# qasimyu/simuscop

Hardware: AMD Instinct MI355X
Metric: simulated paired reads/sec (whole node) at 30x WGS PE150 (higher is better)
Workload: dtype u32

## Files before the change

simuscop_amd/csrc/sg_emit.h:

```cpp
#pragma once
#include "sg_device.h"
#include "sg_philox.h"

namespace sg {

#define EMIT_THREADS 1024
#define EMIT_WAVES (EMIT_THREADS / 64)
#define META_ROW 32

namespace row {
constexpr uint32_t kFlenMask = 0x3FFFFFFFu, kNpMax = 0xFFFFu, kNevMax = 63u, kHdrMax = 1023u;
constexpr uint32_t pack_x(uint32_t flen, uint32_t bad_block, uint32_t rev) { return flen | (bad_block << 30) | (rev << 31); }
constexpr uint32_t pack_y(uint32_t np, uint32_t nev, uint32_t hdr_len) { return np | (nev << 16) | (hdr_len << 22); }
constexpr uint32_t flen(uint32_t x) { return x & kFlenMask; }
constexpr uint32_t bad_block(uint32_t x) { return (x >> 30) & 1u; }
constexpr bool rev(uint32_t x) { return (x >> 31) != 0u; }
constexpr bool active(uint32_t x) { return (x & 0x7FFFFFFFu) != 0u; }
constexpr uint32_t np(uint32_t y) { return y & kNpMax; }
constexpr uint32_t nev(uint32_t y) { return (y >> 16) & kNevMax; }
constexpr uint32_t hdr_len(uint32_t y) { return y >> 22; }
constexpr uint32_t inv_of(uint32_t np) { return 0xFFFFFFFFu / np + 1u; }
constexpr uint32_t pack_src(uint32_t src_m5, bool rc) { return src_m5 | (rc ? 0x80000000u : 0u); }
constexpr uint32_t src_m5(uint32_t w) { return w & 0x7FFFFFFFu; }
constexpr bool copy_is_rc(uint32_t w) { return (w >> 31) != 0u; }

static_assert(np(pack_y(kNpMax, kNevMax, kHdrMax)) == kNpMax && nev(pack_y(kNpMax, kNevMax, kHdrMax)) == kNevMax &&
              hdr_len(pack_y(kNpMax, kNevMax, kHdrMax)) == kHdrMax, "m1.y: extreme values of all three fields");
static_assert(np(pack_y(kNpMax, 0, 0)) == kNpMax && nev(pack_y(kNpMax, 0, 0)) == 0 && hdr_len(pack_y(0, kNevMax, 0)) == 0 &&
              nev(pack_y(0, 0, kHdrMax)) == 0 && np(pack_y(0, kNevMax, kHdrMax)) == 0, "m1.y: no field leaks into a neighbour");
static_assert(flen(pack_x(kFlenMask, 1, 1)) == kFlenMask && bad_block(pack_x(kFlenMask, 1, 1)) == 1 && rev(pack_x(kFlenMask, 1, 1)),
              "m1.x: flen = 2^30 - 1 with both flag bits");
static_assert(bad_block(pack_x(kFlenMask, 0, 1)) == 0 && !rev(pack_x(kFlenMask, 1, 0)) && active(pack_x(1, 0, 0)) &&
              active(pack_x(0, 1, 0)) && !active(pack_x(0, 0, 1)), "m1.x: the flags are independent; rev alone is not active");
static_assert(src_m5(pack_src(0x7FFFFFFFu, true)) == 0x7FFFFFFFu && copy_is_rc(pack_src(0, true)) && !copy_is_rc(pack_src(0x7FFFFFFFu, false)),
              "m0.y of the straight-line kernel's row");
static_assert(inv_of(1) == 0u && inv_of(151) == 28443493u && inv_of(kNpMax) == 65538u, "ceil(2^32 / np) in 32 bits");
}

struct ReadRow {
  uint4 m0, m1;
  __device__ __forceinline__ static ReadRow load(const uint4* meta, size_t idx) { return ReadRow{meta[idx * 3], meta[idx * 3 + 1]}; }
  __device__ __forceinline__ static ReadRow none() { return ReadRow{make_uint4(0, 0, 0, 0), make_uint4(0, 0, 0, 0)}; }
  __device__ __forceinline__ static uint4 make_m0(uint64_t foff, uint32_t namepos, uint32_t fragcount) {
    return make_uint4((uint32_t)foff, (uint32_t)(foff >> 32), namepos, fragcount);
  }
  __device__ __forceinline__ static uint4 make_m1(uint32_t flen, uint32_t bad_block, uint32_t rev, uint32_t np, uint32_t nev,
                                                  uint32_t hdr_len, uint32_t event) {
    return make_uint4(row::pack_x(flen, bad_block, rev), row::pack_y(np, nev, hdr_len), row::inv_of(np), event);
  }
  __device__ __forceinline__ uint32_t flen() const { return row::flen(m1.x); }
  __device__ __forceinline__ bool rev() const { return row::rev(m1.x); }
  __device__ __forceinline__ uint32_t bad_block() const { return row::bad_block(m1.x); }
  __device__ __forceinline__ bool active() const { return row::active(m1.x); }
  __device__ __forceinline__ uint32_t np() const { return row::np(m1.y); }
// ... 197 lines not shown
```

simuscop_amd/csrc/sg_emit_fast.hip:

```cpp
#include "sg_emit.h"

namespace sg {

__device__ __forceinline__ uint32_t pack4(uint32_t w) {
  return (w | (w >> 6) | (w >> 12) | (w >> 18)) & 0xFFu;
}

typedef uint32_t u32x2 __attribute__((ext_vector_type(2)));
typedef uint32_t u32x4 __attribute__((ext_vector_type(4)));

#define FAST_CTX 192u

#define BITOP_OR_AND 0xF8
#define BITOP_XOR_AND 0x78
#define BITOP_ANDN_OR 0xBA

__device__ __noinline__ uint32_t tail_word(uint32_t slot, uint32_t c, uint32_t h, uint32_t c3b, uint32_t k0, uint32_t k1) {
  uint32_t y[4];
  philox_base(slot, 2u * c + (h >> 2), 1u, c3b, k0, k1, y);
  const uint32_t l = h & 3u;
  return l == 0u ? y[0] : l == 1u ? y[1] : l == 2u ? y[2] : y[3];
}

template <int H>
__device__ __forceinline__ void sample1(uint32_t col_sh, uint32_t col_mask, uint32_t cw, uint32_t wh, uint32_t so_h, uint32_t qo_h, uint32_t cd4_w,
                                        uint32_t& acc, uint32_t& sy) {
  typedef const __attribute__((address_space(3))) uint32_t* lds_word;
  const uint32_t kv4 = (cw >> (2 * H + 4)) & 0xFCu;
  const uint32_t keepm1 = *(lds_word)(uintptr_t)(so_h + kv4);
  const uint32_t d_s = keepm1 - (wh >> 16);
  const uint32_t col16 = (wh >> col_sh) & col_mask;
  const uint32_t qa = qo_h + ((cd4_w >> (8 * (H & 3))) & 0xFFu);
  const uint32_t e = *(lds_word)(uintptr_t)(qa + col16 + FAST_CTX * 4u);
  const uint32_t d_q = (wh & 0xFFFFu) - (e & 0xFFFFu);
  const uint32_t z = __builtin_amdgcn_bitop3_b32(d_q - 1u, d_q, d_s, BITOP_ANDN_OR);
  acc = __builtin_amdgcn_bitop3_b32(acc, z, 1u << (17 + H), BITOP_OR_AND);
  sy = __builtin_amdgcn_bitop3_b32(e >> 8, e, d_q, BITOP_XOR_AND);
}

__device__ __forceinline__ void sample8(const uint32_t* code4, uint32_t lgW, uint32_t cw, const uint32_t (&x)[8],
                                        const uint32_t (&so)[8], uint32_t qo0, uint32_t qo1, uint32_t (&sw)[2], uint32_t (&qw)[2],
                                        uint32_t& acc_out) {
  const uint32_t cd4[2] = {code4[(cw >> 10) & 0xFFu], code4[(cw >> 18) & 0xFFu]};
  const uint32_t col_sh = 12u - lgW, col_mask = ((1u << lgW) - 1u) << 4;
  uint32_t acc = 0, sy[8];
  sample1<0>(col_sh, col_mask, cw, x[0], so[0], qo0, cd4[0], acc, sy[0]);
  sample1<1>(col_sh, col_mask, cw, x[1], so[1], qo1, cd4[0], acc, sy[1]);
  sample1<2>(col_sh, col_mask, cw, x[2], so[2], so[2], cd4[0], acc, sy[2]);
  sample1<3>(col_sh, col_mask, cw, x[3], so[3], so[3], cd4[0], acc, sy[3]);
  sample1<4>(col_sh, col_mask, cw, x[4], so[4], so[4], cd4[1], acc, sy[4]);
  sample1<5>(col_sh, col_mask, cw, x[5], so[5], so[5], cd4[1], acc, sy[5]);
  sample1<6>(col_sh, col_mask, cw, x[6], so[6], so[6], cd4[1], acc, sy[6]);
  sample1<7>(col_sh, col_mask, cw, x[7], so[7], so[7], cd4[1], acc, sy[7]);
#pragma unroll
  for (int g = 0; g < 2; g++) {
    const uint32_t p01 = __builtin_amdgcn_perm(sy[4 * g + 1], sy[4 * g], 0x0C0C0602u);
    const uint32_t p23 = __builtin_amdgcn_perm(sy[4 * g + 3], sy[4 * g + 2], 0x06020C0Cu);
    qw[g] = p01 | p23;
    sw[g] = __builtin_amdgcn_perm(0u, 0x47544341u, cd4[g] >> 2);
  }
  acc_out = acc;
}

__device__ __forceinline__ void store_var(uint8_t* q, uint64_t lo, uint64_t hi, uint32_t n) {
  if (n >= 8u) {
    __builtin_memcpy(q, &lo, 8);
    if (n > 8u) {
      const uint32_t k = 8u * (n - 8u);
      const uint64_t v = (lo >> k) | (hi << (64u - k));
      __builtin_memcpy(q + n - 8u, &v, 8);
    }
  } else if (n >= 4u) {
    const uint32_t a = (uint32_t)lo, b = (uint32_t)(lo >> (8u * (n - 4u)));
    __builtin_memcpy(q, &a, 4);
    if (n > 4u) __builtin_memcpy(q + n - 4u, &b, 4);
  } else if (n >= 2u) {
    const uint16_t a = (uint16_t)lo, b = (uint16_t)(lo >> (8u * (n - 2u)));
    __builtin_memcpy(q, &a, 2);
    if (n > 2u) __builtin_memcpy(q + n - 2u, &b, 2);
  } else if (n == 1u) {
    *q = (uint8_t)lo;
  }
}

constexpr uint32_t FAST_G = 63u;

template <bool PAIRED, bool DIAG>
struct FastBlock {
  const DevProfile& P;
  const DevBatch& B;
  uint32_t m, tm;
  uint32_t dg;
  uint32_t bins, TI, inv_TI, clean_cap;
  uint32_t img_at;
  const uint32_t* lut;
  const uint32_t* code4;
  bool tail_whole;
  uint32_t TIp;
  uint32_t TI16, inv_TI16;

  __device__ __forceinline__ FastBlock(const DevProfile& P_, const DevBatch& B_, uint32_t m_, uint32_t TI_, uint32_t inv_TI_,
                                       uint32_t clean_cap_, uint32_t img_at_, const uint32_t* lut_, const uint32_t* code4_)
      : P(P_), B(B_), m(m_), tm(PAIRED ? m_ : 0u), dg(DIAG ? B_.diag : 0u), bins((uint32_t)P_.bins), TI(TI_), inv_TI(inv_TI_),
        clean_cap(clean_cap_), img_at(img_at_), lut(lut_), code4(code4_) {
    tail_whole = ((uint32_t)P.L & 7u) == 7u && ((uint32_t)P.L + 7u) / 8u == TI;
    TIp = tail_whole ? TI : TI - 1u;
    TI16 = (tail_whole ? TIp - 1u : TIp) >> 1;
    inv_TI16 = TI16 ? (1u << 20) / TI16 + 1u : 0u;
  }
  __device__ __forceinline__ bool rc(bool row_bit) const { return PAIRED ? m == 1u : row_bit; }
  __device__ __forceinline__ uint2 fetch_window(bool row_bit, uint32_t idx) const {
    uint2 v;
    fetch_window(row_bit, idx, v);
    return v;
// ... 22 lines not shown
  __device__ __forceinline__ unsigned long long lanes_below() const { return (1ull << lane) - 1ull; }
};

template <bool PAIRED, bool DIAG>
__device__ __forceinline__ void heads8(const FastBlock<PAIRED, DIAG>& k, uint32_t slot, uint32_t c, uint32_t (&x)[8]) {
  const uint32_t c3b = k.c3b();
  if (k.dg & 8u) {
#pragma unroll
    for (int z = 0; z < 8; z++) x[z] = (slot * 2654435761u) ^ (c * 40503u + z * 0x9E3779B9u);
  } else {
    philox_base(slot, 2u * c, 0, c3b, k.B.k0, k.B.k1, x);
    philox_base(slot, 2u * c + 1u, 0, c3b, k.B.k0, k.B.k1, x + 4);
  }
}

template <class S, class Fetch, class Run>
__device__ __forceinline__ void pipelined_steps(S cur, uint32_t first, uint32_t last, Fetch fetch, Run run) {
  for (uint32_t step = first; step < last; step++) {
    const S nxt = fetch(min(step + 1u, last - 1u));
    run(cur);
    cur = nxt;
  }
}

template <bool PAIRED, bool DIAG>
__device__ __forceinline__ void flush_slow(const FastBlock<PAIRED, DIAG>& k, FastWave& w) {
  const DevBatch& B = k.B;
  const uint32_t m = k.m, lane = w.lane;
  wave_lds_sync();
  uint32_t base = 0;
  if (lane == 0u) base = atomicAdd(B.slowq_count + m, w.nslow);
  base = (uint32_t)__builtin_amdgcn_readfirstlane((int)base);
  for (uint32_t b0 = 0; b0 < w.nslow; b0 += 64u) {
    const uint32_t i = b0 + lane;
    if (i < w.nslow && base + i < B.slowq_cap) {
      const uint32_t e = w.slow_list[i];
      B.slowq[(size_t)m * B.slowq_cap + base + i] = make_uint2(w.g * FAST_G + (e & 0xFFu), e >> 8);
    }
  }
  if (lane == 0u && base + w.nslow > B.slowq_cap) atomicOr((unsigned long long*)(B.totals + 3), 2ull);
  w.nslow = 0;
  wave_lds_sync();
}

template <bool PAIRED, bool DIAG>
__device__ __forceinline__ void flush_fix(const FastBlock<PAIRED, DIAG>& k, FastWave& w) {
  const DevProfile& P = k.P;
  const DevBatch& B = k.B;
  const uint32_t bins = k.bins, lane = w.lane;
  wave_lds_sync();
  __builtin_amdgcn_s_waitcnt(0x0F70);
  const uint32_t lgW = P.lgW, u_mask = (1u << (16u - lgW)) - 1u;
  const uint4* gsub = P.fast_sub + (size_t)k.tm * bins * FAST_CTX;
  const uint32_t c3b = k.c3b();
  for (uint32_t b0 = 0; b0 < w.nfix; b0 += 64u) {
    const uint2 fe = w.fix_list[b0 + lane < w.nfix ? b0 + lane : 0u];
    uint32_t todo = b0 + lane < w.nfix ? (fe.x >> 6) & 0xFFu : 0u;
    const uint32_t r = fe.x & 63u, c = fe.x >> 17, cw = fe.y;
    const uint32_t slot = w.g * FAST_G + r + B.slot_offset;
    const FastRow rr = w.rows.load(r);
    const uint32_t np = rr.np(), hl = rr.hdr_len();
    const bool whole = 8u * c + 8u <= np + (uint32_t)((np & 7u) == 7u);
    const uint32_t inv = row::inv_of(max(np, 1u));
    while (__ballot(todo != 0u) != 0ull) {
      const bool on = todo != 0u;
      const uint32_t h = on ? (uint32_t)__builtin_ctz(todo) : 0u;
      todo &= todo - 1u;
      const uint32_t i = 8u * c + h;
      const uint32_t bin = __umulhi(__umul24(i, bins), inv);
      uint32_t xw[4];
      philox_base(slot, 2u * c + (h >> 2), 0, c3b, B.k0, B.k1, xw);
      const uint32_t l = h & 3u;
      const uint32_t wh = l == 0u ? xw[0] : l == 1u ? xw[1] : l == 2u ? xw[2] : xw[3];
      const uint32_t region = c == 0u ? (h == 0u ? 128u : h == 1u ? 64u : 0u) : 0u;
      const uint32_t cdn = (cw >> (2u * h + 10u)) & 3u;
      const uint4 row = gsub[(size_t)bin * FAST_CTX + region + ((cw >> (2u * h + 6u)) & 63u)];
      const uint32_t sh = wh >> 16, h0 = row.x >> 16, h1 = row.y >> 16, h2 = row.z >> 16;
      const uint32_t jj = (uint32_t)(sh > h0) + (uint32_t)(sh > h1) + (uint32_t)(sh > h2);
      const bool amb_s = on && jj != (uint32_t)(sh >= h0) + (uint32_t)(sh >= h1) + (uint32_t)(sh >= h2);
      uint32_t kn = 0;
      uint2 e2 = make_uint2(0, 0);
      const uint32_t col = (wh & 0xFFFFu) >> (16u - lgW), uh = wh & u_mask;
      auto column = [&](uint32_t j_) {
        const uint32_t jm = max(j_, row.w & 3u);
        kn = (row.w >> (2u * jm + 2u)) & 3u;
        e2 = P.fast_alias[((((size_t)cdn * 4u + kn) * bins + bin) << lgW) + col];
      };
      if (!amb_s) column(jj);
      const bool need_tail = amb_s || (on && uh == (e2.x >> 16) && (e2.y & 0xFFu) != (e2.y >> 8));
      uint32_t wt = 0;
      if (__ballot(need_tail) != 0ull) {
        if (need_tail) wt = tail_word(slot, c, h, c3b, B.k0, B.k1);
      }
      if (__ballot(amb_s) != 0ull) {
        if (amb_s) {
          const uint32_t xs = (wh & 0xFFFF0000u) | (wt >> 16);
          column((uint32_t)(xs > row.x) + (uint32_t)(xs > row.y) + (uint32_t)(xs > row.z));
        }
      }
      const uint32_t th = e2.x >> 16;
      const bool lo_side = uh != th ? uh < th : ((uh << 16) | (wt & 0xFFFFu)) < e2.x;
      const uint32_t sym = (lo_side ? (e2.y & 0xFFu) : (e2.y >> 8)) + (uint32_t)P.min_qual;
      const uint32_t ch = (0x47544341u >> (8u * kn)) & 0xFFu;
      if (on) {
        if (whole) {
          uint8_t* rec = w.gout + rr.out_off() + hl + i;
          rec[0] = (uint8_t)ch;
          rec[np + 3u] = (uint8_t)sym;
        } else if (!rr.parked_slow()) {
          w.rows.patch_parked(r, h, ch, sym);
        }
      }
    }
  }
  w.nfix = 0;
  wave_lds_sync();
}

template <bool PAIRED, bool DIAG>
__device__ __forceinline__ void push_fix(const FastBlock<PAIRED, DIAG>& k, FastWave& w, uint32_t r, uint32_t c, uint32_t fix, uint32_t cw) {
  const unsigned long long fm = __ballot(fix != 0u);
  if (fm) {
    if (w.nfix + 64u > FIX_CAP) flush_fix(k, w);
    if (fix != 0u) w.fix_list[w.nfix + (uint32_t)__popcll(fm & w.lanes_below())] = make_uint2(r | (fix << 6) | (c << 17), cw);
    w.nfix += (uint32_t)__popcll(fm);
  }
}

__device__ __forceinline__ void stage_tables(const DevProfile& P, uint32_t tm, uint32_t TI, uint32_t* img, uint32_t img_at,
                                             uint32_t* lut, uint32_t* code4) {
  const uint32_t tid = threadIdx.x, bins = (uint32_t)P.bins, img_words = bins * P.fast_stride;
  const uint4* src = (const uint4*)(P.fast_lds + (size_t)tm * P.fast_mate_words);
  for (uint32_t i = tid; i < (img_words + 3u) / 4u; i += EMIT_THREADS) ((uint4*)img)[i] = src[i];
  const uint32_t blk_bytes = P.fast_stride * 4u;
  for (uint32_t i = tid; i < TI * LUT_ROW; i += EMIT_THREADS) {
    const uint32_t c = i / LUT_ROW, f = i - c * LUT_ROW;
    const uint32_t h = f < 8u ? f : f - 8u;
    const uint32_t pos = 8u * c + h;
    const uint32_t bin = min(pos * bins / (uint32_t)P.L, bins - 1u);
    uint32_t v = bin * blk_bytes;
    if (f < 8u && c == 0u) v += f == 0u ? 128u * 4u : f == 1u ? 64u * 4u : 0u;
    lut[i] = f < 10u ? v + img_at : 0u;
  }
  for (uint32_t i = tid; i < 256u; i += EMIT_THREADS) {
    uint32_t v = 0;
    for (uint32_t z = 0; z < 4u; z++) v |= (((i >> (2u * z)) & 3u) * 4u) << (8u * z);
    code4[i] = v;
  }
}

template <bool PAIRED>
__device__ __forceinline__ void store_name(const DevBatch& B, uint32_t m, const ReadRow& my, size_t idx, uint8_t* rec) {
  const uint32_t nv = my.hdr_len() - B.prefix_len;
  if (__builtin_expect(nv > 16u, 0)) {
    write_name(rec, B.prefix, B.prefix_len, my.namepos(), my.fragcount(), PAIRED ? 1u : 0u, m);
    return;
  }
  const uint64_t p_lo = ((uint64_t)B.prefix_w[1] << 32) | B.prefix_w[0], p_hi = ((uint64_t)B.prefix_w[3] << 32) | B.prefix_w[2];
  const uint4 tx = B.meta[idx * 3 + 2];
  const uint64_t b0 = ((uint64_t)tx.y << 32) | tx.x, b1 = ((uint64_t)tx.w << 32) | tx.z;
  const uint32_t plen = B.prefix_len, hb = plen + nv;
  if (plen < 16u && hb >= 16u && hb <= 24u) {
    const uint32_t sh = 8u * plen;
    uint64_t w0, w1, w2;
    if (sh < 64u) {
      w0 = p_lo | (b0 << sh);
      w1 = p_hi | (b1 << sh) | (sh ? b0 >> (64u - sh) : 0ull);
      w2 = sh ? b1 >> (64u - sh) : 0ull;
    } else {
      const uint32_t t2 = sh - 64u;
      w0 = p_lo;
      w1 = p_hi | (b0 << t2);
      w2 = (b1 << t2) | (t2 ? b0 >> (64u - t2) : 0ull);
    }
    struct { uint64_t a, b; } first = {w0, w1};
    __builtin_memcpy(rec, &first, 16);
    const uint32_t n2 = hb - 16u;
// ... 110 lines not shown
  {
    const uint32_t rem = gp.n_clean & 63u, idle = (0u - (gp.n_fast * TI + gp.n_single + gp.n_gen_all)) & 63u;
    if (rem != 0u && rem <= idle && gp.n_single + gp.n_gen_all + rem <= OVF_CAP) gp.n_moved = rem;
  }
  gp.n_ovf = gp.n_moved + gp.n_single + gp.n_gen_all;
  gp.more = (k.dg & 256u) ? 0ull : __ballot(gp.extra > 2u);
  return gp;
}

template <bool PAIRED, bool DIAG>
__device__ __forceinline__ void compose_lists(const FastBlock<PAIRED, DIAG>& k, const FastWave& w, GroupPlan& gp) {
  const uint32_t TI = k.TI, lane = w.lane, items = gp.items, n_moved = gp.n_moved;
  const unsigned long long lt = w.lanes_below();
  if (items > 0u && !gp.split_l) {
    if (gp.plain_l) {
      const uint32_t pos = (uint32_t)__popcll(gp.m_plain & lt);
      w.permp[pos] = (uint8_t)lane;
      if (!k.tail_whole) w.ovf[n_moved + pos] = (uint16_t)(lane | (k.TIp << 8));
    } else {
      uint32_t pos;
      if ((gp.m_rest >> lane) & 1ull) pos = (uint32_t)__popcll(gp.m_rest & lt);
      else if ((gp.m_one >> lane) & 1ull) pos = gp.n_rest + (uint32_t)__popcll(gp.m_one & lt);
      else pos = gp.n_rest + gp.n_one + (uint32_t)__popcll(gp.m_multi & lt);
      w.perm[pos] = (uint8_t)lane;
    }
  }
  if (gp.n_fast == 0u && lane == 0u) w.perm[0] = 0;
  if (gp.small) {
    const uint32_t o = n_moved + gp.n_psingle + (uint32_t)__popcll(gp.b1 & lt) + (uint32_t)__popcll(gp.b2 & lt);
    w.ovf[o] = (uint16_t)(lane | (TI << 8));
    if (gp.extra == 2u) w.ovf[o + 1u] = (uint16_t)(lane | ((TI + 1u) << 8));
  }
  if (gp.split_l) {
    const uint32_t kb = gp.kb, ka = gp.ka, ca0 = gp.ca0;
    const uint32_t oc = (gp.vscan >> 16) - (kb + ka);
    uint32_t og = n_moved + gp.n_single + (gp.vscan & 0xFFFFu) - gp.n_gen;
    const uint32_t kt = kb + ka, behind = ((ca0 - kb) << 7) | 64u;
    for (uint32_t q = 0; q < kt; q++) w.clean[oc + q] = (uint16_t)((lane | (q << 7)) + (q >= kb ? behind : 0u));
    const uint32_t mid_end = ka ? ca0 : items;
    for (uint32_t c = kb; c < mid_end; c++) w.ovf[og++] = (uint16_t)(lane | (c << 8));
    if (ka) for (uint32_t c = gp.n_whole; c < items; c++) w.ovf[og++] = (uint16_t)(lane | (c << 8));
  }
  wave_lds_sync();
  if (n_moved) {
    gp.n_clean -= n_moved;
    if (lane < n_moved) {
      const uint32_t e = w.clean[gp.n_clean + lane];
      w.ovf[lane] = (uint16_t)((e & 63u) | ((e >> 7) << 8));
    }
    wave_lds_sync();
  }
}

struct PlainSteps {
  bool use16;
  uint32_t n_plain, np16steps, cnt8, c8_base, n_pitems, npsteps;
};
template <bool PAIRED, bool DIAG>
__device__ __forceinline__ PlainSteps plan_plain_steps(const FastBlock<PAIRED, DIAG>& k, uint32_t n_plain) {
  PlainSteps ps;
  const uint32_t dg = k.dg, TIp = k.TIp, TI16 = k.TI16;
  ps.n_plain = n_plain;
  ps.use16 = !(dg & 512u) && TIp >= 18u;
  const uint32_t n_p16 = ps.use16 ? n_plain * TI16 : 0u;
  ps.np16steps = (dg & 128u) ? 0u : n_p16 >> 6;
  const uint32_t rem16 = n_p16 - (ps.np16steps << 6);
  ps.cnt8 = ps.use16 ? TIp - 2u * TI16 : TIp;
  ps.c8_base = ps.use16 ? 2u * TI16 : 0u;
  ps.n_pitems = 2u * rem16 + n_plain * ps.cnt8;
  ps.npsteps = (dg & 128u) ? 0u : (ps.n_pitems + 63u) / 64u;
  return ps;
}

__device__ __forceinline__ void lut_bins(const uint32_t* lut, uint32_t c, uint32_t (&so)[8], uint32_t& qo0, uint32_t& qo1) {
  const uint4* lrow = (const uint4*)(lut + c * LUT_ROW);
  const uint4 r0 = lrow[0], r1 = lrow[1], r2 = lrow[2];
  so[0] = r0.x; so[1] = r0.y; so[2] = r0.z; so[3] = r0.w; so[4] = r1.x; so[5] = r1.y; so[6] = r1.z; so[7] = r1.w;
  qo0 = r2.x; qo1 = r2.y;
}

struct P16 { uint32_t r, c, src, out; uint2 w; };

template <bool PAIRED, bool DIAG>
__device__ __forceinline__ void plain16_step(const FastBlock<PAIRED, DIAG>& k, FastWave& w, const P16& st, uint32_t qual_at) {
  const uint32_t dg = k.dg;
  const uint32_t c8 = 2u * st.c;
  const uint64_t w64 = window_codes(st.w, st.src);
  uint32_t cwa = (uint32_t)w64, cwb = (uint32_t)(w64 >> 16);
  const uint32_t slot = w.g * FAST_G + st.r + k.B.slot_offset;
  if (dg & 4u) { cwa = (w.g * FAST_G + st.r) * 2654435761u + c8; cwb = cwa * 40503u + 1u; }
  uint32_t sw[4], qw[4], fixv[2];
#pragma unroll
  for (int hf = 0; hf < 2; hf++) {
    uint32_t x[8];
    const uint32_t c = c8 + (uint32_t)hf, cw = hf ? cwb : cwa;
    heads8(k, slot, c, x);
    uint32_t so[8], qo0, qo1;
    lut_bins(k.lut, c, so, qo0, qo1);
    uint32_t s2[2], q2[2], acc;
    sample8(k.code4, k.P.lgW, cw, x, so, qo0, qo1, s2, q2, acc);
    sw[2 * hf] = s2[0]; sw[2 * hf + 1] = s2[1];
    qw[2 * hf] = q2[0]; qw[2 * hf + 1] = q2[1];
    fixv[hf] = (dg & 16u) ? 0u : (acc >> 17) & 0xFFu;
  }
  const uint32_t so_ = (dg & 1u) ? 0xFFFFFFFFu : st.out;
  const uint32_t qo_ = (dg & 1u) ? 0xFFFFFFFFu : st.out + qual_at;
  __builtin_amdgcn_raw_buffer_store_b128(u32x4{sw[0], sw[1], sw[2], sw[3]}, w.out_rsrc, so_, 0, 0);
  __builtin_amdgcn_raw_buffer_store_b128(u32x4{qw[0], qw[1], qw[2], qw[3]}, w.out_rsrc, qo_, 0, 0);
#pragma unroll
  for (int hf = 0; hf < 2; hf++) push_fix(k, w, st.r, c8 + (uint32_t)hf, fixv[hf], hf ? cwb : cwa);
}

template <bool PAIRED, bool DIAG>
__device__ __forceinline__ void plain16_steps(const FastBlock<PAIRED, DIAG>& k, FastWave& w, uint32_t a16, uint32_t b16) {
  uint32_t TI16_v = k.TI16, inv_TI16_v = k.inv_TI16, qual_at = (uint32_t)k.P.L + 3u;
  asm volatile("" : "+v"(TI16_v), "+v"(inv_TI16_v), "+v"(qual_at));
  auto fetch16 = [&](uint32_t step) -> P16 {
    P16 st;
    const uint32_t i = step * 64u + w.lane;
    const uint32_t ri = __umul24(i, inv_TI16_v) >> 20;
    st.c = i - __umul24(ri, TI16_v);
    st.r = w.permp[ri];
    const uint32_t A = w.rows.src_word(st.r);
    st.src = row::src_m5(A) + 16u * st.c;
    st.out = w.rows.base_off(st.r) + 16u * st.c;
    st.w = k.fetch_window(row::copy_is_rc(A), st.src);
    return st;
  };
  P16 cur = fetch16(a16);
  __builtin_amdgcn_raw_buffer_store_b128(u32x4{0u, 0u, 0u, 0u}, w.out_rsrc, 0xFFFFFFFFu, 0, 0);
  __builtin_amdgcn_raw_buffer_store_b128(u32x4{0u, 0u, 0u, 0u}, w.out_rsrc, 0xFFFFFFF0u, 0, 0);
  pipelined_steps(cur, a16, b16, fetch16, [&](const P16& st) { plain16_step(k, w, st, qual_at); });
}

template <bool PAIRED, bool DIAG>
__device__ __forceinline__ void sample_store8(const FastBlock<PAIRED, DIAG>& k, FastWave& w, uint32_t r, uint32_t c, bool ok, uint2 win,
                                              uint32_t src, const uint32_t (&so)[8], uint32_t qo0, uint32_t qo1, uint32_t out,
                                              uint32_t qual_at, bool tail_patch) {
  const uint32_t dg = k.dg;
  uint32_t cw;
  if (dg & 4u) cw = (w.g * FAST_G + r) * 2654435761u + c;
  else cw = (uint32_t)window_codes(win, src);
  uint32_t x[8];
  heads8(k, w.g * FAST_G + r + k.B.slot_offset, c, x);
  uint32_t sw[2], qw[2], acc;
  sample8(k.code4, k.P.lgW, cw, x, so, qo0, qo1, sw, qw, acc);
  const bool st_ok = ok && !(dg & 1u);
  const uint32_t so_ = st_ok ? out : 0xFFFFFFFFu;
  const uint32_t qo_ = st_ok ? out + qual_at : 0xFFFFFFFFu;
  uint32_t fix_mask = 0xFFu;
  if (tail_patch) {
    const bool last = c + 1u == k.TI;
    const uint32_t sel = last ? 0x04020100u : 0x03020100u;
    sw[1] = __builtin_amdgcn_perm(0x0Au, sw[1], sel);
    qw[1] = __builtin_amdgcn_perm(0x0Au, qw[1], sel);
    __builtin_amdgcn_raw_buffer_store_b16((unsigned short)0x0A2Bu, w.out_rsrc, st_ok && last ? so_ + 8u : 0xFFFFFFFFu, 0, 0);
    fix_mask = last ? 0x7Fu : 0xFFu;
  }
  __builtin_amdgcn_raw_buffer_store_b64(u32x2{sw[0], sw[1]}, w.out_rsrc, so_, 0, 0);
  __builtin_amdgcn_raw_buffer_store_b64(u32x2{qw[0], qw[1]}, w.out_rsrc, qo_, 0, 0);
  const uint32_t fix = (ok && !(dg & 16u)) ? (acc >> 17) & fix_mask : 0u;
  push_fix(k, w, r, c, fix, cw);
}

struct PStage { uint32_t r, c, src, out; bool ok; uint2 w; };

template <bool PAIRED, bool DIAG>
__device__ __forceinline__ void plain8_steps(const FastBlock<PAIRED, DIAG>& k, FastWave& w, const PlainSteps& ps, uint32_t a8, uint32_t b8) {
  const uint32_t cnt8 = ps.cnt8, c8_base = ps.c8_base, n_pitems = ps.n_pitems, TI16 = k.TI16, inv_TI16 = k.inv_TI16;
  uint32_t qual_at = (uint32_t)k.P.L + 3u, n_single = ps.n_plain * cnt8, i16_base = ps.np16steps << 6;
  asm volatile("" : "+v"(qual_at), "+v"(n_single), "+v"(i16_base));
  const uint32_t inv_cnt8 = cnt8 ? (1u << 20) / cnt8 + 1u : 0u;
  auto fetch_plain = [&](uint32_t step) -> PStage {
    PStage st;
    const uint32_t i_raw = step * 64u + w.lane;
    st.ok = i_raw < n_pitems;
    const uint32_t i = min(i_raw, n_pitems - 1u);
    const bool half = i >= n_single;
    const uint32_t j = i - n_single;
    const uint32_t q = half ? i16_base + (j >> 1) : i;
    const uint32_t d = half ? TI16 : cnt8;
    const uint32_t ri = __umul24(q, half ? inv_TI16 : inv_cnt8) >> 20;
    const uint32_t rem = q - __umul24(ri, d);
    st.c = half ? 2u * rem + (j & 1u) : c8_base + rem;
    st.r = w.permp[ri];
    const uint32_t A = w.rows.src_word(st.r);
    st.src = row::src_m5(A) + 8u * st.c;
    st.out = w.rows.base_off(st.r) + 8u * st.c;
    st.w = k.fetch_window(row::copy_is_rc(A), st.src);
    return st;
  };
  auto run_plain = [&](const PStage& st) {
    uint32_t so[8], qo0, qo1;
    lut_bins(k.lut, st.c, so, qo0, qo1);
    sample_store8(k, w, st.r, st.c, st.ok, st.w, st.src, so, qo0, qo1, st.out, qual_at, k.tail_whole);
  };
  PStage cur = fetch_plain(a8);
  __builtin_amdgcn_raw_buffer_store_b64(u32x2{0u, 0u}, w.out_rsrc, 0xFFFFFFFFu, 0, 0);
  __builtin_amdgcn_raw_buffer_store_b64(u32x2{0u, 0u}, w.out_rsrc, 0xFFFFFFF0u, 0, 0);
  if (k.tail_whole) __builtin_amdgcn_raw_buffer_store_b16((unsigned short)0u, w.out_rsrc, 0xFFFFFFE0u, 0, 0);
  pipelined_steps(cur, a8, b8, fetch_plain, run_plain);
}

template <bool PAIRED, bool DIAG>
__device__ __forceinline__ void plain_steps(const FastBlock<PAIRED, DIAG>& k, FastWave& w, uint32_t n_plain) {
  const PlainSteps ps = plan_plain_steps(k, n_plain);
  const uint32_t h16 = ps.np16steps >> 1, s8_first = (ps.use16 && ps.cnt8 && ps.npsteps) ? 1u : 0u;
#pragma unroll 1
  for (uint32_t ph = 0; ph < 2u; ph++) {
    const uint32_t a16 = ph ? h16 : 0u, b16 = ph ? ps.np16steps : h16;
    const uint32_t a8 = ph ? s8_first : 0u, b8 = ph ? ps.npsteps : s8_first;
    if (a16 < b16) plain16_steps(k, w, a16, b16);
    if (a8 < b8) plain8_steps(k, w, ps, a8, b8);
  }
}
// ... 136 lines not shown
    }
#pragma unroll 1
    for (; __ballot(q_ins <= q_end) != 0ull; q_ins++) {
      if (q_ins <= q_end) {
        const int p = (int)i0 - 5 + q_ins, ej = (int)(ie.ew_in & 0xFFFFu);
        const uint32_t prof = __umulhi(aux_draw(k.B, slot, ie.tj_in, (uint32_t)(p - ej), k.m), 3u);
        const uint32_t nat = (k.P.inv_remap_packed >> (2u * prof)) & 3u;
        cw = (cw & ~(3u << (2 * q_ins))) | (nat << (2 * q_ins));
      }
    }
  }
  return cw;
}

template <bool PAIRED, bool DIAG>
__device__ __forceinline__ void item_bins(const FastBlock<PAIRED, DIAG>& k, const Stage& st, uint32_t (&so)[8], uint32_t& qo0, uint32_t& qo1) {
  const uint32_t c = st.c, bins = k.bins, blk_bytes = k.P.fast_stride * 4u;
  const bool active = st.active;
  const bool lut_ok = st.row.np() == (uint32_t)k.P.L && c < k.TI;
  if (__ballot(active && !lut_ok) == 0ull) {
    lut_bins(k.lut, lut_ok ? c : 0u, so, qo0, qo1);
  } else {
    const uint32_t ib0 = __umul24(8u * c, bins), inv = st.row.inv();
#pragma unroll
    for (int h = 0; h < 8; h++) {
      const uint32_t bin = __umulhi(ib0 + (uint32_t)h * bins, inv);
      so[h] = __umul24(active ? bin : 0u, blk_bytes) + k.img_at;
    }
    qo0 = so[0]; qo1 = so[1];
    if (c == 0u) { so[0] += 128u * 4u; so[1] += 64u * 4u; }
  }
}

template <bool PAIRED, bool DIAG>
__device__ __forceinline__ void store_item(const FastBlock<PAIRED, DIAG>& k, const FastWave& w, const Stage& st, bool slow,
                                           const uint32_t (&sw)[2], const uint32_t (&qw)[2]) {
  const uint32_t np = st.row.np(), i0 = 8u * st.c;
  const bool active = st.active, go = active && !slow;
  const bool last7 = i0 + 7u == np;
  const bool whole = i0 + 8u <= np || last7;
  const bool sto = go && whole && !(k.dg & 1u);
  const uint32_t so_ = sto ? st.row.out_off() + st.row.hdr_len() + i0 : 0xFFFFFFFFu;
  const uint32_t qo_ = sto ? so_ + np + 3u : 0xFFFFFFFFu;
  const uint32_t s1 = last7 ? (sw[1] & 0x00FFFFFFu) | 0x0A000000u : sw[1];
  const uint32_t q1 = last7 ? (qw[1] & 0x00FFFFFFu) | 0x0A000000u : qw[1];
  __builtin_amdgcn_raw_buffer_store_b64(u32x2{sw[0], s1}, w.out_rsrc, so_, 0, 0);
  __builtin_amdgcn_raw_buffer_store_b64(u32x2{qw[0], q1}, w.out_rsrc, qo_, 0, 0);
  __builtin_amdgcn_raw_buffer_store_b16((unsigned short)0x0A2Bu, w.out_rsrc, sto && last7 ? so_ + 8u : 0xFFFFFFFFu, 0, 0);
  if (active && i0 + 8u > np && !(last7 && !slow)) w.rows.park(st.r, slow, sw, qw);
}

template <bool PAIRED, bool DIAG>
__device__ __forceinline__ bool fast_item(const FastBlock<PAIRED, DIAG>& k, const FastWave& w, const Stage& st, const ItemEvents& ie,
                                          uint32_t& fix, uint32_t& cw_out) {
  const bool active = st.active;
  const uint32_t c = st.c, slot = w.g * FAST_G + st.r;
  const uint32_t np = st.row.np(), nev = active ? ie.n_in : 0u;
  const uint32_t bad = st.row.bad_block();
  const uint32_t cw = item_codes(k, st, st.w, ie, nev, slot);
  uint32_t x[8];
  heads8(k, slot + k.B.slot_offset, c, x);
  uint32_t so[8], qo0, qo1;
  item_bins(k, st, so, qo0, qo1);
  uint32_t qw[2], sw[2], acc;
  sample8(k.code4, k.P.lgW, cw, x, so, qo0, qo1, sw, qw, acc);
  const bool slow = active && (bad != 0u || nev >= 2u);
  fix = (active && !slow && !(k.dg & 16u)) ? (acc >> 17) & 0xFFu & ((1u << min(8u, np - 8u * c)) - 1u) : 0u;
  cw_out = cw;
  store_item(k, w, st, slow, sw, qw);
  return slow;
}

template <bool PAIRED, bool DIAG>
__device__ __forceinline__ void general_step(const FastBlock<PAIRED, DIAG>& k, FastWave& w, const Stage& st) {
  const ItemEvents ie = item_events(k, w, st);
  uint32_t fix, cw;
  const bool slow = fast_item(k, w, st, ie, fix, cw);
  const unsigned long long sm = __ballot(slow);
  if (sm) {
    if (slow) w.slow_list[w.nslow + (uint32_t)__popcll(sm & w.lanes_below())] = st.r | (st.c << 8);
    w.nslow += (uint32_t)__popcll(sm);
  }
  push_fix(k, w, st.r, st.c, fix, cw);
}

template <bool PAIRED, bool DIAG>
__device__ __forceinline__ void general_steps(const FastBlock<PAIRED, DIAG>& k, FastWave& w, const GroupPlan& gp) {
  const uint32_t n_items = gp.n_fast * k.TI, n_stream = n_items + gp.n_ovf;
  const uint32_t nmain = (k.dg & 256u) ? 0u : (n_stream + 63u) / 64u;
  if (!nmain) return;
  Stage cur = fetch_step(k, w, n_items, n_stream, 0u);
  __builtin_amdgcn_raw_buffer_store_b64(u32x2{0u, 0u}, w.out_rsrc, 0xFFFFFFFFu, 0, 0);
  __builtin_amdgcn_raw_buffer_store_b64(u32x2{0u, 0u}, w.out_rsrc, 0xFFFFFFF0u, 0, 0);
  __builtin_amdgcn_raw_buffer_store_b16((unsigned short)0u, w.out_rsrc, 0xFFFFFFE0u, 0, 0);
  pipelined_steps(
      cur, 0u, nmain,
      [&](uint32_t step) {
        if (w.nslow > SLOW_CAP - 64u) flush_slow(k, w);
        return fetch_step(k, w, n_items, n_stream, step);
      },
      [&](const Stage& st) { general_step(k, w, st); });
}

template <bool PAIRED, bool DIAG>
__device__ __forceinline__ void past_map_steps(const FastBlock<PAIRED, DIAG>& k, FastWave& w, unsigned long long more) {
  uint32_t cb = k.TI;
  while (more) {
    if (w.nslow > SLOW_CAP - 64u) flush_slow(k, w);
    const uint32_t r = (uint32_t)__builtin_ctzll(more);
    const uint32_t c = cb + w.lane;
    const uint32_t nitems = (w.rows.np(r) + 7u) / 8u;
    cb += 64u;
    if (cb >= nitems) { more &= more - 1ull; cb = k.TI; }
    const Stage st = fetch_item(k, w, r, c, true, 1u);
    general_step(k, w, st);
  }
}

__device__ __forceinline__ void tail_pass(const FastWave& w) {
  const FastRow r = w.rows.load(w.lane);
  if (!r.active()) return;
  const uint32_t np = r.np(), hl = r.hdr_len();
  uint8_t* rec = w.gout + r.out_off();
  if ((np & 7u) == 7u && !r.parked_slow()) {
  } else {
    const uint32_t d = !r.parked_slow() ? (np & 7u) : 0u;
    const uint64_t S = r.parked_bases(), Q = r.parked_quals();
    const uint64_t keep = (1ull << (8u * d)) - 1ull;
    uint8_t* so = rec + hl + (np - d);
    const uint64_t s_lo = (S & keep) | (0x0A2B0Aull << (8u * d));
    const uint64_t s_hi = d > 5u ? (0x0A2B0Aull >> (8u * (8u - d))) : 0ull;
    store_var(so, s_lo, s_hi, d + 3u);
    store_var(so + np + 3u, (Q & keep) | (0x0Aull << (8u * d)), 0ull, d + 1u);
  }
}

// ... 99 lines not shown
```

Measured before the change: 2.330 billion.

## Reduce fast-path fix-up detection to one undecided flag per item, recompute lanes in flush

The hot sampling path no longer builds an 8-bit per-base fix mask. It computes a single 'undecided' predicate per item by OR-ing the keep deltas and taking the minimum of the quality deltas. Fix-up entries now carry only the read, item and window codes, and for 16-base plain steps one entry covers both halves. flush_fix recomputes the per-base flags by re-running the sampling in a new flagged8 routine before resolving them. Hot-loop ALU and fix-list pushes shrink, at the price of redundant recomputation in the rare fix-up flush and a new packed entry format.

```diff
diff --git a/simuscop_amd/csrc/sg_emit.h b/simuscop_amd/csrc/sg_emit.h
--- a/simuscop_amd/csrc/sg_emit.h
+++ b/simuscop_amd/csrc/sg_emit.h
@@ -1,5 +1,6 @@
 #pragma once
 #include "sg_device.h"
+#include "sg_fix_entry.h"
 #include "sg_philox.h"
 
 namespace sg {
diff --git a/simuscop_amd/csrc/sg_emit_fast.hip b/simuscop_amd/csrc/sg_emit_fast.hip
--- a/simuscop_amd/csrc/sg_emit_fast.hip
+++ b/simuscop_amd/csrc/sg_emit_fast.hip
@@ -14,6 +14,7 @@
 #define BITOP_OR_AND 0xF8
 #define BITOP_XOR_AND 0x78
 #define BITOP_ANDN_OR 0xBA
+#define BITOP_OR3 0xFE
 
 __device__ __noinline__ uint32_t tail_word(uint32_t slot, uint32_t c, uint32_t h, uint32_t c3b, uint32_t k0, uint32_t k1) {
   uint32_t y[4];
@@ -24,34 +25,41 @@
 
 template <int H>
 __device__ __forceinline__ void sample1(uint32_t col_sh, uint32_t col_mask, uint32_t cw, uint32_t wh, uint32_t so_h, uint32_t qo_h, uint32_t cd4_w,
-                                        uint32_t& acc, uint32_t& sy) {
+                                        uint32_t& d_s, uint32_t& d_q, uint32_t& sy) {
   typedef const __attribute__((address_space(3))) uint32_t* lds_word;
   const uint32_t kv4 = (cw >> (2 * H + 4)) & 0xFCu;
   const uint32_t keepm1 = *(lds_word)(uintptr_t)(so_h + kv4);
-  const uint32_t d_s = keepm1 - (wh >> 16);
+  d_s = keepm1 - (wh >> 16);
   const uint32_t col16 = (wh >> col_sh) & col_mask;
   const uint32_t qa = qo_h + ((cd4_w >> (8 * (H & 3))) & 0xFFu);
   const uint32_t e = *(lds_word)(uintptr_t)(qa + col16 + FAST_CTX * 4u);
-  const uint32_t d_q = (wh & 0xFFFFu) - (e & 0xFFFFu);
-  const uint32_t z = __builtin_amdgcn_bitop3_b32(d_q - 1u, d_q, d_s, BITOP_ANDN_OR);
-  acc = __builtin_amdgcn_bitop3_b32(acc, z, 1u << (17 + H), BITOP_OR_AND);
+  d_q = (wh & 0xFFFFu) - (e & 0xFFFFu);
   sy = __builtin_amdgcn_bitop3_b32(e >> 8, e, d_q, BITOP_XOR_AND);
 }
 
 __device__ __forceinline__ void sample8(const uint32_t* code4, uint32_t lgW, uint32_t cw, const uint32_t (&x)[8],
-                                        const uint32_t (&so)[8], uint32_t qo0, uint32_t qo1, uint32_t (&sw)[2], uint32_t (&qw)[2],
-                                        uint32_t& acc_out) {
+                                        const uint32_t (&so)[8], uint32_t qo0, uint32_t qo1, uint32_t skip7, uint32_t (&sw)[2],
+                                        uint32_t (&qw)[2], uint32_t& undecided) {
   const uint32_t cd4[2] = {code4[(cw >> 10) & 0xFFu], code4[(cw >> 18) & 0xFFu]};
   const uint32_t col_sh = 12u - lgW, col_mask = ((1u << lgW) - 1u) << 4;
-  uint32_t acc = 0, sy[8];
-  sample1<0>(col_sh, col_mask, cw, x[0], so[0], qo0, cd4[0], acc, sy[0]);
-  sample1<1>(col_sh, col_mask, cw, x[1], so[1], qo1, cd4[0], acc, sy[1]);
-  sample1<2>(col_sh, col_mask, cw, x[2], so[2], so[2], cd4[0], acc, sy[2]);
-  sample1<3>(col_sh, col_mask, cw, x[3], so[3], so[3], cd4[0], acc, sy[3]);
-  sample1<4>(col_sh, col_mask, cw, x[4], so[4], so[4], cd4[1], acc, sy[4]);
-  sample1<5>(col_sh, col_mask, cw, x[5], so[5], so[5], cd4[1], acc, sy[5]);
-  sample1<6>(col_sh, col_mask, cw, x[6], so[6], so[6], cd4[1], acc, sy[6]);
-  sample1<7>(col_sh, col_mask, cw, x[7], so[7], so[7], cd4[1], acc, sy[7]);
+  uint32_t ds[8], dq[8], sy[8];
+  sample1<0>(col_sh, col_mask, cw, x[0], so[0], qo0, cd4[0], ds[0], dq[0], sy[0]);
+  sample1<1>(col_sh, col_mask, cw, x[1], so[1], qo1, cd4[0], ds[1], dq[1], sy[1]);
+  sample1<2>(col_sh, col_mask, cw, x[2], so[2], so[2], cd4[0], ds[2], dq[2], sy[2]);
+  sample1<3>(col_sh, col_mask, cw, x[3], so[3], so[3], cd4[0], ds[3], dq[3], sy[3]);
+  sample1<4>(col_sh, col_mask, cw, x[4], so[4], so[4], cd4[1], ds[4], dq[4], sy[4]);
+  sample1<5>(col_sh, col_mask, cw, x[5], so[5], so[5], cd4[1], ds[5], dq[5], sy[5]);
+  sample1<6>(col_sh, col_mask, cw, x[6], so[6], so[6], cd4[1], ds[6], dq[6], sy[6]);
+  sample1<7>(col_sh, col_mask, cw, x[7], so[7], so[7], cd4[1], ds[7], dq[7], sy[7]);
+  {
+    const uint32_t s012 = __builtin_amdgcn_bitop3_b32(ds[0], ds[1], ds[2], BITOP_OR3);
+    const uint32_t s01234 = __builtin_amdgcn_bitop3_b32(s012, ds[3], ds[4], BITOP_OR3);
+    const uint32_t s0_6 = __builtin_amdgcn_bitop3_b32(s01234, ds[5], ds[6], BITOP_OR3);
+    const uint32_t s_any = s0_6 | (ds[7] & ~skip7);
+    const uint32_t q012 = min(min(dq[0], dq[1]), dq[2]), q01234 = min(min(q012, dq[3]), dq[4]);
+    const uint32_t q_min = min(min(min(q01234, dq[5]), dq[6]), dq[7] | skip7);
+    undecided = __builtin_amdgcn_bitop3_b32(q_min - 1u, q_min, s_any, BITOP_ANDN_OR);
+  }
 #pragma unroll
   for (int g = 0; g < 2; g++) {
     const uint32_t p01 = __builtin_amdgcn_perm(sy[4 * g + 1], sy[4 * g], 0x0C0C0602u);
@@ -59,7 +67,25 @@
     qw[g] = p01 | p23;
     sw[g] = __builtin_amdgcn_perm(0u, 0x47544341u, cd4[g] >> 2);
   }
-  acc_out = acc;
+}
+
+__device__ __forceinline__ uint32_t flagged8(const uint32_t* code4, uint32_t lgW, uint32_t cw, const uint32_t (&x)[8],
+                                             const uint32_t (&so)[8], uint32_t qo0, uint32_t qo1) {
+  const uint32_t cd4[2] = {code4[(cw >> 10) & 0xFFu], code4[(cw >> 18) & 0xFFu]};
+  const uint32_t col_sh = 12u - lgW, col_mask = ((1u << lgW) - 1u) << 4;
+  uint32_t ds[8], dq[8], sy;
+  sample1<0>(col_sh, col_mask, cw, x[0], so[0], qo0, cd4[0], ds[0], dq[0], sy);
+  sample1<1>(col_sh, col_mask, cw, x[1], so[1], qo1, cd4[0], ds[1], dq[1], sy);
+  sample1<2>(col_sh, col_mask, cw, x[2], so[2], so[2], cd4[0], ds[2], dq[2], sy);
+  sample1<3>(col_sh, col_mask, cw, x[3], so[3], so[3], cd4[0], ds[3], dq[3], sy);
+  sample1<4>(col_sh, col_mask, cw, x[4], so[4], so[4], cd4[1], ds[4], dq[4], sy);
+  sample1<5>(col_sh, col_mask, cw, x[5], so[5], so[5], cd4[1], ds[5], dq[5], sy);
+  sample1<6>(col_sh, col_mask, cw, x[6], so[6], so[6], cd4[1], ds[6], dq[6], sy);
+  sample1<7>(col_sh, col_mask, cw, x[7], so[7], so[7], cd4[1], ds[7], dq[7], sy);
+  uint32_t f = 0;
+#pragma unroll
+  for (int h = 0; h < 8; h++) f |= (uint32_t)((int32_t)ds[h] < 0 || dq[h] == 0u) << h;
+  return f;
 }
 
 __device__ __forceinline__ void store_var(uint8_t* q, uint64_t lo, uint64_t hi, uint32_t n) {
@@ -188,20 +214,46 @@
   __builtin_amdgcn_s_waitcnt(0x0F70);
   const uint32_t lgW = P.lgW, u_mask = (1u << (16u - lgW)) - 1u;
   const uint4* gsub = P.fast_sub + (size_t)k.tm * bins * FAST_CTX;
-  const uint32_t c3b = k.c3b();
+  const uint32_t c3b = k.c3b(), blk_bytes = P.fast_stride * 4u;
   for (uint32_t b0 = 0; b0 < w.nfix; b0 += 64u) {
-    const uint2 fe = w.fix_list[b0 + lane < w.nfix ? b0 + lane : 0u];
-    uint32_t todo = b0 + lane < w.nfix ? (fe.x >> 6) & 0xFFu : 0u;
-    const uint32_t r = fe.x & 63u, c = fe.x >> 17, cw = fe.y;
+    const bool have = b0 + lane < w.nfix;
+    const uint2 raw = w.fix_list[have ? b0 + lane : 0u];
+    const fixent::Entry fe{raw.x, raw.y};
+    const uint32_t r = fixent::read(fe), hm = fixent::halves(fe);
+    const uint64_t codes = fixent::codes(fe);
+    const uint32_t c0 = hm ? 2u * fixent::item(fe) : fixent::item(fe);
+    const uint32_t want = have ? (hm ? hm : 1u) : 0u;
     const uint32_t slot = w.g * FAST_G + r + B.slot_offset;
     const FastRow rr = w.rows.load(r);
     const uint32_t np = rr.np(), hl = rr.hdr_len();
-    const bool whole = 8u * c + 8u <= np + (uint32_t)((np & 7u) == 7u);
     const uint32_t inv = row::inv_of(max(np, 1u));
+    uint32_t todo = 0;
+#pragma unroll 1
+    for (uint32_t hf = 0; hf < 2u; hf++) {
+      const bool on_hf = ((want >> hf) & 1u) != 0u;
+      if (__ballot(on_hf) == 0ull) continue;
+      const uint32_t c = c0 + hf, cw = (uint32_t)(codes >> (16u * hf));
+      uint32_t x[8], so[8];
+      heads8(k, slot, c, x);
+      const uint32_t ib0 = __umul24(8u * c, bins);
+#pragma unroll
+      for (int h = 0; h < 8; h++) so[h] = __umul24(__umulhi(ib0 + (uint32_t)h * bins, inv), blk_bytes) + k.img_at;
+      const uint32_t qo0 = so[0], qo1 = so[1];
+      if (c == 0u) { so[0] += 128u * 4u; so[1] += 64u * 4u; }
+      const uint32_t f = on_hf ? flagged8(k.code4, lgW, cw, x, so, qo0, qo1) : 0u;
+      if (DIAG) {
+        const uint32_t n_none = (uint32_t)__popcll(__ballot(on_hf && f == 0u));
+        if (n_none && lane == 0u) atomicAdd((unsigned long long*)(B.totals + 5), (unsigned long long)n_none);
+      }
+      const uint32_t n_here = np > 8u * c ? min(8u, np - 8u * c) : 0u;
+      todo |= (f & ((1u << n_here) - 1u)) << (8u * hf);
+    }
     while (__ballot(todo != 0u) != 0ull) {
       const bool on = todo != 0u;
-      const uint32_t h = on ? (uint32_t)__builtin_ctz(todo) : 0u;
+      const uint32_t h16 = on ? (uint32_t)__builtin_ctz(todo) : 0u;
       todo &= todo - 1u;
+      const uint32_t c = c0 + (h16 >> 3), h = h16 & 7u, cw = (uint32_t)(codes >> (2u * (h16 & 8u)));
+      const bool whole = 8u * c + 8u <= np + (uint32_t)((np & 7u) == 7u);
       const uint32_t i = 8u * c + h;
       const uint32_t bin = __umulhi(__umul24(i, bins), inv);
       uint32_t xw[4];
@@ -254,11 +306,15 @@
 }
 
 template <bool PAIRED, bool DIAG>
-__device__ __forceinline__ void push_fix(const FastBlock<PAIRED, DIAG>& k, FastWave& w, uint32_t r, uint32_t c, uint32_t fix, uint32_t cw) {
-  const unsigned long long fm = __ballot(fix != 0u);
+__device__ __forceinline__ void push_fix(const FastBlock<PAIRED, DIAG>& k, FastWave& w, bool flagged, uint32_t r, uint32_t halves,
+                                         uint32_t item, uint64_t codes) {
+  const unsigned long long fm = __ballot(flagged);
   if (fm) {
     if (w.nfix + 64u > FIX_CAP) flush_fix(k, w);
-    if (fix != 0u) w.fix_list[w.nfix + (uint32_t)__popcll(fm & w.lanes_below())] = make_uint2(r | (fix << 6) | (c << 17), cw);
+    if (flagged) {
+      const fixent::Entry e = fixent::pack(r, halves, item, codes);
+      w.fix_list[w.nfix + (uint32_t)__popcll(fm & w.lanes_below())] = make_uint2(e.x, e.y);
+    }
     w.nfix += (uint32_t)__popcll(fm);
   }
 }
@@ -475,6 +531,7 @@
   }
 }
 
+static_assert(64u / 2u <= fixent::kItemMax + 1u, "every 16-base item index of the lane map fits the fix-up entry");
 struct PlainSteps {
   bool use16;
   uint32_t n_plain, np16steps, cnt8, c8_base, n_pitems, npsteps;
@@ -508,11 +565,11 @@
 __device__ __forceinline__ void plain16_step(const FastBlock<PAIRED, DIAG>& k, FastWave& w, const P16& st, uint32_t qual_at) {
   const uint32_t dg = k.dg;
   const uint32_t c8 = 2u * st.c;
-  const uint64_t w64 = window_codes(st.w, st.src);
-  uint32_t cwa = (uint32_t)w64, cwb = (uint32_t)(w64 >> 16);
+  uint64_t w64 = window_codes(st.w, st.src);
   const uint32_t slot = w.g * FAST_G + st.r + k.B.slot_offset;
-  if (dg & 4u) { cwa = (w.g * FAST_G + st.r) * 2654435761u + c8; cwb = cwa * 40503u + 1u; }
-  uint32_t sw[4], qw[4], fixv[2];
+  if (dg & 4u) w64 = (uint64_t)((w.g * FAST_G + st.r) * 2654435761u + c8) * 40503u;
+  const uint32_t cwa = (uint32_t)w64, cwb = (uint32_t)(w64 >> 16);
+  uint32_t sw[4], qw[4], und[2];
 #pragma unroll
   for (int hf = 0; hf < 2; hf++) {
     uint32_t x[8];
@@ -520,18 +577,17 @@
     heads8(k, slot, c, x);
     uint32_t so[8], qo0, qo1;
     lut_bins(k.lut, c, so, qo0, qo1);
-    uint32_t s2[2], q2[2], acc;
-    sample8(k.code4, k.P.lgW, cw, x, so, qo0, qo1, s2, q2, acc);
+    uint32_t s2[2], q2[2];
+    sample8(k.code4, k.P.lgW, cw, x, so, qo0, qo1, 0u, s2, q2, und[hf]);
     sw[2 * hf] = s2[0]; sw[2 * hf + 1] = s2[1];
     qw[2 * hf] = q2[0]; qw[2 * hf + 1] = q2[1];
-    fixv[hf] = (dg & 16u) ? 0u : (acc >> 17) & 0xFFu;
   }
   const uint32_t so_ = (dg & 1u) ? 0xFFFFFFFFu : st.out;
   const uint32_t qo_ = (dg & 1u) ? 0xFFFFFFFFu : st.out + qual_at;
   __builtin_amdgcn_raw_buffer_store_b128(u32x4{sw[0], sw[1], sw[2], sw[3]}, w.out_rsrc, so_, 0, 0);
   __builtin_amdgcn_raw_buffer_store_b128(u32x4{qw[0], qw[1], qw[2], qw[3]}, w.out_rsrc, qo_, 0, 0);
-#pragma unroll
-  for (int hf = 0; hf < 2; hf++) push_fix(k, w, st.r, c8 + (uint32_t)hf, fixv[hf], hf ? cwb : cwa);
+  const uint32_t halves = (dg & 16u) ? 0u : (und[0] >> 31) | ((und[1] >> 30) & 2u);
+  push_fix(k, w, halves != 0u, st.r, halves, st.c, w64);
 }
 
 template <bool PAIRED, bool DIAG>
@@ -566,24 +622,21 @@
   else cw = (uint32_t)window_codes(win, src);
   uint32_t x[8];
   heads8(k, w.g * FAST_G + r + k.B.slot_offset, c, x);
-  uint32_t sw[2], qw[2], acc;
-  sample8(k.code4, k.P.lgW, cw, x, so, qo0, qo1, sw, qw, acc);
+  uint32_t sw[2], qw[2], und;
+  const bool last = tail_patch && c + 1u == k.TI;
+  sample8(k.code4, k.P.lgW, cw, x, so, qo0, qo1, last ? 0xFFFFFFFFu : 0u, sw, qw, und);
   const bool st_ok = ok && !(dg & 1u);
   const uint32_t so_ = st_ok ? out : 0xFFFFFFFFu;
   const uint32_t qo_ = st_ok ? out + qual_at : 0xFFFFFFFFu;
-  uint32_t fix_mask = 0xFFu;
   if (tail_patch) {
-    const bool last = c + 1u == k.TI;
     const uint32_t sel = last ? 0x04020100u : 0x03020100u;
     sw[1] = __builtin_amdgcn_perm(0x0Au, sw[1], sel);
     qw[1] = __builtin_amdgcn_perm(0x0Au, qw[1], sel);
     __builtin_amdgcn_raw_buffer_store_b16((unsigned short)0x0A2Bu, w.out_rsrc, st_ok && last ? so_ + 8u : 0xFFFFFFFFu, 0, 0);
-    fix_mask = last ? 0x7Fu : 0xFFu;
   }
   __builtin_amdgcn_raw_buffer_store_b64(u32x2{sw[0], sw[1]}, w.out_rsrc, so_, 0, 0);
   __builtin_amdgcn_raw_buffer_store_b64(u32x2{qw[0], qw[1]}, w.out_rsrc, qo_, 0, 0);
-  const uint32_t fix = (ok && !(dg & 16u)) ? (acc >> 17) & fix_mask : 0u;
-  push_fix(k, w, r, c, fix, cw);
+  push_fix(k, w, ok && !(dg & 16u) && (int32_t)und < 0, r, 0u, c, cw);
 }
 
 struct PStage { uint32_t r, c, src, out; bool ok; uint2 w; };
@@ -826,20 +879,20 @@
 
 template <bool PAIRED, bool DIAG>
 __device__ __forceinline__ bool fast_item(const FastBlock<PAIRED, DIAG>& k, const FastWave& w, const Stage& st, const ItemEvents& ie,
-                                          uint32_t& fix, uint32_t& cw_out) {
+                                          bool& fix, uint32_t& cw_out) {
   const bool active = st.active;
   const uint32_t c = st.c, slot = w.g * FAST_G + st.r;
-  const uint32_t np = st.row.np(), nev = active ? ie.n_in : 0u;
+  const uint32_t nev = active ? ie.n_in : 0u;
   const uint32_t bad = st.row.bad_block();
   const uint32_t cw = item_codes(k, st, st.w, ie, nev, slot);
   uint32_t x[8];
   heads8(k, slot + k.B.slot_offset, c, x);
   uint32_t so[8], qo0, qo1;
   item_bins(k, st, so, qo0, qo1);
-  uint32_t qw[2], sw[2], acc;
-  sample8(k.code4, k.P.lgW, cw, x, so, qo0, qo1, sw, qw, acc);
+  uint32_t qw[2], sw[2], und;
+  sample8(k.code4, k.P.lgW, cw, x, so, qo0, qo1, 0u, sw, qw, und);
   const bool slow = active && (bad != 0u || nev >= 2u);
-  fix = (active && !slow && !(k.dg & 16u)) ? (acc >> 17) & 0xFFu & ((1u << min(8u, np - 8u * c)) - 1u) : 0u;
+  fix = active && !slow && !(k.dg & 16u) && (int32_t)und < 0;
   cw_out = cw;
   store_item(k, w, st, slow, sw, qw);
   return slow;
@@ -848,14 +901,15 @@
 template <bool PAIRED, bool DIAG>
 __device__ __forceinline__ void general_step(const FastBlock<PAIRED, DIAG>& k, FastWave& w, const Stage& st) {
   const ItemEvents ie = item_events(k, w, st);
-  uint32_t fix, cw;
+  bool fix;
+  uint32_t cw;
   const bool slow = fast_item(k, w, st, ie, fix, cw);
   const unsigned long long sm = __ballot(slow);
   if (sm) {
     if (slow) w.slow_list[w.nslow + (uint32_t)__popcll(sm & w.lanes_below())] = st.r | (st.c << 8);
     w.nslow += (uint32_t)__popcll(sm);
   }
-  push_fix(k, w, st.r, st.c, fix, cw);
+  push_fix(k, w, fix, st.r, 0u, st.c, cw);
 }
 
 template <bool PAIRED, bool DIAG>
diff --git a/simuscop_amd/csrc/sg_fix_entry.h b/simuscop_amd/csrc/sg_fix_entry.h
--- /dev/null
+++ b/simuscop_amd/csrc/sg_fix_entry.h
@@ -0,0 +1,35 @@
+#pragma once
+#include <stdint.h>
+
+namespace sg {
+namespace fixent {
+
+constexpr uint32_t kReadBits = 6, kHalfBits = 2, kItemBits = 14, kCodeHiBits = 10;
+constexpr uint32_t kHalfShift = kReadBits, kItemShift = kReadBits + kHalfBits, kCodeHiShift = kItemShift + kItemBits;
+constexpr uint32_t kReadMax = (1u << kReadBits) - 1u, kItemMax = (1u << kItemBits) - 1u;
+constexpr uint32_t kCodeBits = 32u + kCodeHiBits;
+constexpr uint64_t kCodeMask = (1ull << kCodeBits) - 1ull;
+
+static_assert(kReadBits + kHalfBits + kItemBits + kCodeHiBits == 32, "the first word's four fields fill it");
+static_assert(kCodeBits == 2 * 21, "a 16-base item's window: 21 codes");
+static_assert(kReadMax >= 62, "a group has 63 reads");
+static_assert(65535u / 8u <= kItemMax, "every 8-base item of a read of 65535 bases");
+
+struct Entry { uint32_t x, y; };
+
+constexpr Entry pack(uint32_t read, uint32_t halves, uint32_t item, uint64_t codes) {
+  return Entry{read | (halves << kHalfShift) | (item << kItemShift) | ((uint32_t)(codes >> 32) << kCodeHiShift), (uint32_t)codes};
+}
+constexpr uint32_t read(Entry e) { return e.x & kReadMax; }
+constexpr uint32_t halves(Entry e) { return (e.x >> kHalfShift) & ((1u << kHalfBits) - 1u); }
+constexpr uint32_t item(Entry e) { return (e.x >> kItemShift) & kItemMax; }
+constexpr uint64_t codes(Entry e) { return ((uint64_t)(e.x >> kCodeHiShift) << 32) | e.y; }
+
+static_assert(read(pack(62, 3, kItemMax, kCodeMask)) == 62 && halves(pack(62, 3, kItemMax, kCodeMask)) == 3 &&
+              item(pack(62, 3, kItemMax, kCodeMask)) == kItemMax && codes(pack(62, 3, kItemMax, kCodeMask)) == kCodeMask,
+              "every field at its extreme");
+static_assert(read(pack(0, 0, 0, kCodeMask)) == 0 && halves(pack(0, 0, 0, kCodeMask)) == 0 && item(pack(0, 0, 0, kCodeMask)) == 0 &&
+              codes(pack(kReadMax, 3, kItemMax, 0)) == 0 && codes(pack(0, 0, 0, ~0ull)) == kCodeMask, "no field leaks into a neighbour");
+
+}
+}
```

New measurement: 2.262 billion. 0.971x the previous value.
